# AlibabaResearch/efficientteacher

Measured on AMD Instinct MI355X. Metric: SSOD images/sec (teacher+student step) YOLOv5l 640px, higher is better.
Workload: dtype bf16

## Files before the change

efficientteacher_amd/_lib.py:

```python
import ctypes
import os
from ctypes import c_char_p, c_double, c_float, c_int, c_int64, c_size_t, c_void_p

import torch

_HERE = os.path.dirname(os.path.abspath(__file__))
LIB_PATH = os.environ.get("ET_HIP_LIB") or os.path.join(_HERE, "libet_hip.so")

ET_F32, ET_BF16, ET_F16 = 0, 1, 2

P = c_void_p
SIGNATURES = {
    "et_build_arch": (c_char_p, []),
    "et_abi_version": (c_int, []),
    "et_nms_ssod_workspace_bytes": (c_int, [c_int, c_int, ctypes.POINTER(c_size_t)]),
    "et_nms_workspace_bytes": (c_int, [c_int, c_int, c_int, c_int, c_int, ctypes.POINTER(c_size_t)]),
    "et_nms": (c_int, [P, c_int, c_int, c_int, c_float, c_float, c_int, c_int, ctypes.c_uint64, ctypes.c_uint64, c_int,
                       c_float, c_int, P, P, P, P, P, c_size_t, P]),
    "et_nms_ssod": (c_int, [P, c_int, c_int, c_int, c_float, c_float, c_int, c_int, P, P, P, P, P, c_size_t, P]),
    "et_val_match": (c_int, [P, c_int, P, c_int, c_int, P, c_int, P, c_int, c_int, P, c_int, c_int, c_int, c_int64, c_int64,
                             P, P, P, P, P, P]),
    "et_val_ap_workspace_bytes": (c_int, [c_int, ctypes.POINTER(c_size_t)]),
    "et_val_ap": (c_int, [P, P, P, c_int64, P, c_int, c_int, P, P, P, P, P, c_size_t, P]),
    "et_detect_decode": (c_int, [P, c_int, c_int, c_int, c_int, c_int, c_int, c_int64, c_int64, c_int64, c_int64,
                                 P, c_float, P, c_int64, c_int64, P]),
    "et_ema_update": (c_int, [P, P, c_int64, c_float, c_float, P]),
    "et_adamw": (c_int, [P, P, P, P, P, c_int, c_int64, c_float, c_float, c_float, c_float, c_float, c_int, c_float, P, P]),
    "et_adamw_tick": (c_int, [P, c_float, c_float, P, P]),
    "et_adamw_dev": (c_int, [P, P, P, P, P, c_int, c_int64, c_float, c_float, c_float, c_float, c_float, P, c_float, P, P]),
    "et_sgd_nesterov": (c_int, [P, P, P, P, c_int, c_int64, c_float, c_float, c_float, c_int, c_float, P, P]),
    "et_cast_f32_to_lp": (c_int, [P, P, c_int, c_int64, P]),
    "et_scaler_check": (c_int, [P, c_int64, P, P]),
    "et_scaler_update": (c_int, [P, c_float, c_float, c_int, P]),
    "et_ema_update_dev": (c_int, [P, P, c_int64, P, P]),
    "et_sgd_nesterov_dev": (c_int, [P, P, P, P, c_int, c_int64, P, c_int, P, P]),
    "et_conv2d_stats_rows": (c_int, [c_int, c_int, c_int]),
    "et_conv2d_stats_rows_for": (c_int, [c_int] * 12),
    "et_conv2d_stats_adds_for": (c_int, [c_int] * 12),
    "et_conv2d_fwd": (c_int, [P, P, P, c_int] + [c_int] * 11 + [P, P, c_int, P, c_int, P, c_int, P, P]),
    "et_conv2d_dgrad": (c_int, [P, P, P, c_int] + [c_int] * 11 + [c_int, P, c_int, P, P]),
    "et_conv2d_dgrad_bn": (c_int, [P, P, P, c_int] + [c_int] * 10 + [P, c_int, P, c_int, P, P, c_int, P, c_int, P, P]),
    "et_conv2d_wgrad": (c_int, [P, P, P, c_int] + [c_int] * 11 + [P, P]),
    "et_conv2d_wgrad_grouped": (c_int, [P, c_int, c_int] + [c_int] * 9 + [P, P]),
    "et_weight_transpose_all": (c_int, [P, P, c_int, P, c_int, ctypes.c_longlong, P]),
    "et_weight_transpose": (c_int, [P, P, c_int, c_int, c_int, c_int, P]),
    "et_conv2d_kernel_name": (c_int, [c_int] * 13 + [c_char_p, c_int]),
    "et_env_knobs": (c_int, [c_char_p, c_int]),
    "et_colsum": (c_int, [P, c_int, c_int, c_int, c_int, P, P]),
    "et_bn_reduce_rows": (c_int, [c_int, c_int, c_int]),
    "et_bn_finalize": (c_int, [P, c_int, c_int, c_double, P, P, c_float, c_float, P, P, P, P, P, P, P, P]),
    "et_bn_eval_affine": (c_int, [c_int, P, P, P, P, c_float, P, P, P]),
    "et_bn_act_fwd": (c_int, [P, c_int, P, c_int, P, c_int, c_int, c_int, c_int, P, P, c_int, P]),
    "et_bn_act_fwd_sharded": (c_int, [P, c_int, P, c_int, P, c_int, c_int, c_int, c_int, P, c_int, c_double, P, P, c_float, c_float,
                                      P, P, P, P, P, P, c_int, P]),
    "et_bn_act_bwd_sharded": (c_int, [P, c_int, P, c_int, P, c_int, c_int, c_int, c_int, P, P, P, P, P, c_int, P, P, P, c_int, c_int, P]),
    "et_bn_act_bwd": (c_int, [P, c_int, P, c_int, P, c_int, c_int, c_int, c_int, P, P, P, P, P, c_int, P, P, P, P,
                              c_size_t, P]),
    "et_bn_act_bwd_from_partials": (c_int, [P, c_int, P, c_int, P, c_int, c_int, c_int, c_int, P, P, P, P, P, c_int, P, P, P,
                                            P, c_int, P, P]),
    "et_act_bwd": (c_int, [P, c_int, P, c_int, P, c_int, c_int, c_int, c_int, c_int, P]),
    "et_pack_input": (c_int, [P, P, c_int, c_int, c_int, c_int, c_int, P]),
    "et_pack_input_u8": (c_int, [P, P, c_int, c_int, c_int, c_int, c_int, c_float, P]),
    "et_maxpool5_fwd": (c_int, [P, c_int, P, c_int, P, c_int, c_int, c_int, c_int, c_int, P]),
    "et_maxpool5_bwd": (c_int, [P, c_int, P, P, c_int, P, c_int, c_int, c_int, c_int, c_int, c_int, P]),
    "et_upsample2x_fwd": (c_int, [P, c_int, P, c_int, c_int, c_int, c_int, c_int, c_int, P]),
    "et_upsample2x_bwd": (c_int, [P, c_int, P, c_int, c_int, c_int, c_int, c_int, c_int, c_int, P]),
    "et_strong_view_u8": (c_int, [P, P, c_int, c_int, c_int, P, P, P, P, c_int, P]),
    "et_mosaic4_u8": (c_int, [P, P, c_int, c_int, c_int, P]),
# ... 6 lines not shown
    "et_scale_cast": (c_int, [P, P, c_int, c_int64, c_float, P, P]),
    "et_domain_focal": (c_int, [P, c_int, c_int, c_int64, c_int, c_float, P, c_int, P, P]),
    "et_scale_inplace": (c_int, [P, c_int, c_int64, c_float, P, P]),
    "et_v8_decode": (c_int, [P, c_int, P, c_int, c_int, c_int, c_int, c_int, c_int, c_int, c_float, c_float, P, c_int64, c_int64, P]),
    "et_tal_loss": (c_int, [P, P, P, P, P, P, P, c_int, c_int, c_int, c_int, c_int, c_float, c_float, c_float, P, P, P, P, P]),
    "et_tal_assign_workspace_bytes": (c_int, [c_int, c_int, c_int, ctypes.POINTER(c_size_t)]),
    "et_tal_assign": (c_int, [P, P, P, P, P, P, c_int, c_int, c_int, c_int, c_int, c_float, c_float, c_float, P, P, P, P, P, c_size_t, P]),
    "et_tal_targets_pad": (c_int, [P, c_int, c_int, c_int, c_float, c_float, P, P, P]),
    "et_tal_pseudo_split": (c_int, [P, P, P, P, c_int, c_int, c_int, c_int, c_int, c_int, c_float, c_float, P, P, P, P, P, P, P, P, P]),
    "et_tal_assigned_gt": (c_int, [P, c_int, c_int, c_int, P, P]),
    "et_tal_merge_pseudo": (c_int, [P, P, P, P, P, P, P, P, P, c_int, c_int, c_int, c_int, P, P, P, P]),
}



class WgradItem(ctypes.Structure):
    _fields_ = [("x", ctypes.c_void_p), ("dy", ctypes.c_void_p), ("dw", ctypes.c_void_p), ("ldx", ctypes.c_int),
                ("ldy", ctypes.c_int)]


class LossLevel(ctypes.Structure):
    _fields_ = [("p", P), ("dp", P), ("tobj_ws", P), ("sb", c_int64), ("sa", c_int64), ("sy", c_int64),
                ("sx", c_int64), ("ny", c_int), ("nx", c_int), ("anchors", c_float * 6), ("balance", c_float)]


class LossDesc(ctypes.Structure):
    _fields_ = [("dtype", c_int), ("B", c_int), ("na", c_int), ("nc", c_int), ("NT", c_int), ("nl", c_int),
                ("anchor_t", c_float), ("gr", c_float), ("cp", c_float), ("cn", c_float), ("cls_pw", c_float),
                ("obj_pw", c_float), ("box_w", c_float), ("obj_w", c_float), ("cls_w", c_float),
                ("pass_mask", c_int), ("ignore_obj", c_int), ("targets", P), ("acc_ws", P), ("out", P),
                ("ota_match", P), ("obj_channel", c_int), ("balance_dev", P), ("autobalance_ssi", c_int), ("fl_gamma", c_float), ("level", LossLevel * 4)]


_dll = None
_emulated = False
CALL_TIMER = None
_NO_LAUNCH = frozenset(n for n in (
    "et_build_arch", "et_abi_version", "et_nms_ssod_workspace_bytes", "et_nms_workspace_bytes", "et_conv2d_stats_rows", "et_conv2d_stats_rows_for",
    "et_conv2d_kernel_name", "et_env_knobs", "et_bn_reduce_rows", "et_ota_workspace_bytes", "et_tal_assign_workspace_bytes", "et_val_ap_workspace_bytes"))


class _TimedDll:

    def __init__(self, dll, timer):
        self._dll, self._timer, self._cache = dll, timer, {}

    def __getattr__(self, name):
        fn = self._cache.get(name)
        if fn is None:
            raw = getattr(self._dll, name)
            if name in _NO_LAUNCH or not name.startswith("et_"):
                fn = raw
            else:
                timer = self._timer

                def fn(*a, _raw=raw, _name=name):
                    tok = timer.begin(_name)
                    rc = _raw(*a)
                    timer.end(tok)
                    return rc
            self._cache[name] = fn
        return fn


class EtHipError(RuntimeError):
    pass
# ... 78 lines not shown
```

efficientteacher_amd/csrc/conv.hip:

```cpp
#include "et_device.h"
#include "../../include/et_hip.h"
#include <stdlib.h>
#include <stdio.h>
#include <string.h>
#include <type_traits>

typedef __attribute__((ext_vector_type(16))) float f32x16;
typedef __attribute__((ext_vector_type(8))) __bf16 bf16x8;
typedef __attribute__((ext_vector_type(8))) _Float16 f16x8;
typedef __attribute__((ext_vector_type(4))) unsigned int u32x4;
__device__ __forceinline__ u32x4 mk4(unsigned a, unsigned b, unsigned c, unsigned d) { u32x4 v = {a, b, c, d}; return v; }
__device__ __forceinline__ void et_pin_loaded(u32x4& v) {
#if defined(__HIP_DEVICE_COMPILE__)
    asm volatile("" : "+v"(v));
#endif
}

template <typename T, typename V> __device__ __forceinline__ f32x16 et_mfma32(const V a, const V b, const f32x16 c) {
    static_assert(sizeof(V) == 16, "8 x 16-bit operands");
    if constexpr (std::is_same<T, et_f16>::value)
        return __builtin_amdgcn_mfma_f32_32x32x16_f16(__builtin_bit_cast(f16x8, a), __builtin_bit_cast(f16x8, b), c, 0, 0, 0);
    else
        return __builtin_amdgcn_mfma_f32_32x32x16_bf16(__builtin_bit_cast(bf16x8, a), __builtin_bit_cast(bf16x8, b), c, 0, 0, 0);
}
// ... 3031 lines not shown
extern "C" int et_conv2d_kernel_name(int op, int dtype, int N, int IH, int IW, int Cin, int Cout, int KH, int KW, int stride,
                                     int pad, int have_zero_page, int parity_class, char* buf, int buflen) {
    if (!buf || buflen < 8) return -1;
    if (KH * KW > CONV_MAX_TAPS || stride < 1 || N <= 0) return -2;
    const int eb = dtype == ET_F32 ? 4 : 2, vec = dtype == ET_F32 ? 4 : 8;
    if (op == 2) {
        WgradGeom g;
        wgrad_geom(g, N, IH, IW, Cin, Cin, Cout, KH, KW, stride, pad, Cout);
        wgrad_plan_name(plan_wgrad(g, eb, have_zero_page != 0), dtype, buf, buflen);
        return 0;
    }
    GatherGeom g;
    const bool full = op == 3 || op == 4;
    if (op == 3) op = 1;
    if (op == 4) op = 0;
    if (op == 0) {
        if (!full && try_launch_stem(nullptr, nullptr, nullptr, dtype, N, IH, IW, Cin, Cin, Cout, KH, KW, stride, pad, Cout, nullptr, nullptr, 0,
                                     nullptr, nullptr, 0, have_zero_page ? (const void*)buf : nullptr, nullptr, false)) {
            snprintf(buf, buflen, "conv_stem_kernel");
            return 0;
        }
        if (fwd_geom(g, N, IH, IW, Cin, Cin, Cout, KH, KW, stride, pad, Cout, vec)) return -2;
    } else if (op == 1) {
        if (stride > 2 || Cout % vec) return -2;
        const int py = parity_class / stride, px = parity_class % stride;
        if (py >= stride) return -2;
        if (dgrad_geom(g, py, px, N, IH, IW, Cin, Cin, Cout, KH, KW, stride, pad, Cout, vec)) return -2;
    } else return -2;
    plan_name(plan_gemm(g, eb, have_zero_page != 0, full), dtype, buf, buflen);
    return 0;
}

extern "C" int et_env_knobs(char* buf, int buflen) {
    static const char* names[] = {"ET_CONV_S1_WGS", "ET_CONV_STEM_WGS", "ET_CONV_BUF_DMA", "ET_BN_FIN_SMALL", "ET_STEP_GRAPH", "ET_WGRAD_STREAM",
                                  "ET_ALLREDUCE_CHUNK_MB", "ET_ALLREDUCE_DTYPE", "ET_RCCL_CHANNELS", "ET_DP_SINGLE_RANK", "ET_HIP_LIB"};
    if (!buf || buflen < 1) return -1;
    int off = 0;
    buf[0] = 0;
    for (const char* n : names) {
        const char* v = getenv(n);
        if (!v) continue;
        const int w = snprintf(buf + off, buflen - off, "%s=%s;", n, v);
        if (w < 0 || w >= buflen - off) return -3;
        off += w;
    }
    return 0;
}
```

efficientteacher_amd/csrc/optim.hip:

```cpp
#include "et_device.h"
#include <math.h>
#include "../../include/et_hip.h"

__device__ __forceinline__ uint16_t lp_of(float v, int shadow_dtype) { return shadow_dtype == ET_F16 ? et_f2h(v) : et_f2bf(v); }
#define ET_SCALER_SKIP(scaler) ((scaler) != nullptr && (scaler)[2] != 0.0f)
#define ET_SCALER_INV(scaler) ((scaler) != nullptr ? (scaler)[1] : 1.0f)

__global__ __launch_bounds__(256) void ema_kernel(float* __restrict__ v, const float* __restrict__ m, long long n,
                                                  float d, float omd) {
    const long long i4 = ((long long)blockIdx.x * 256 + threadIdx.x) * 4;
    if (i4 + 3 < n) {
        float4 a = *(float4*)(v + i4);
        const float4 b = *(const float4*)(m + i4);
        a.x = a.x * d; a.x = a.x + omd * b.x;
        a.y = a.y * d; a.y = a.y + omd * b.y;
        a.z = a.z * d; a.z = a.z + omd * b.z;
        a.w = a.w * d; a.w = a.w + omd * b.w;
        *(float4*)(v + i4) = a;
    } else {
        for (long long i = i4; i < n; ++i) { float a = v[i] * d; v[i] = a + omd * m[i]; }
    }
}

extern "C" int et_ema_update(float* ema, const float* model, int64_t n, float d, float one_minus_d,
// ... 65 lines not shown
}

__global__ __launch_bounds__(256) void sgd_kernel(float* __restrict__ p, const float* __restrict__ g,
                                                  float* __restrict__ buf, uint16_t* __restrict__ shadow, int shadow_dtype,
                                                  long long n, float lr, float mu, float wd, int first,
                                                  float inv_scale_host, const float* __restrict__ scaler) {
    if (ET_SCALER_SKIP(scaler)) return;
    const float inv_scale = inv_scale_host * ET_SCALER_INV(scaler);
    const long long i = (long long)blockIdx.x * 256 + threadIdx.x;
    if (i >= n) return;
    float gi = g[i] * inv_scale;
    const float pi = p[i];
    if (wd != 0.0f) gi = gi + wd * pi;
    float b = first ? gi : (buf[i] * mu + gi);
    buf[i] = b;
    gi = gi + mu * b;
    const float o = pi - lr * gi;
    p[i] = o;
    if (shadow) shadow[i] = lp_of(o, shadow_dtype);
}

extern "C" int et_sgd_nesterov(float* p, const float* grad, float* momentum_buf, void* lp_shadow, int shadow_dtype, int64_t n,
                               float lr, float momentum, float weight_decay, int first_step, float inv_scale,
                               const float* scaler, et_stream_t stream) {
    if (!p || !grad || !momentum_buf) return -1;
    if (n < 0 || (lp_shadow && shadow_dtype != ET_BF16 && shadow_dtype != ET_F16)) return -2;
    if (n == 0) return 0;
    hipLaunchKernelGGL(sgd_kernel, dim3(et_cdiv(n, 256)), dim3(256), 0, (hipStream_t)stream, p, grad, momentum_buf,
                       (uint16_t*)lp_shadow, shadow_dtype, (long long)n, lr, momentum, weight_decay, first_step, inv_scale, scaler);
    ET_CHECK_LAUNCH();
    return 0;
}

template <bool DEV>
__global__ __launch_bounds__(256) void adamw_kernel(float* __restrict__ p, const float* __restrict__ g, float* __restrict__ m,
                                                    float* __restrict__ v, uint16_t* __restrict__ shadow, int shadow_dtype, long long n,
                                                    float lr_wd, float b1, float b2, float step_size, float inv_sqrt_bc2, float eps,
                                                    float inv_scale_host, const float* __restrict__ scaler, float lr,
                                                    const double* __restrict__ tick) {
    if (ET_SCALER_SKIP(scaler)) return;
    if constexpr (DEV) {
        step_size = (float)((double)lr / tick[1]);
        inv_sqrt_bc2 = (float)(1.0 / sqrt(tick[2]));
    }
    const float inv_scale = inv_scale_host * ET_SCALER_INV(scaler);
    const long long i = (long long)blockIdx.x * 256 + threadIdx.x;
    if (i >= n) return;
    const float gi = g[i] * inv_scale;
    float pi = p[i];
    pi = pi * (1.0f - lr_wd);
    float mi = m[i];
    mi = mi + (gi - mi) * (1.0f - b1);
    float vi = v[i] * b2;
    vi = vi + (1.0f - b2) * gi * gi;
    const float denom = sqrtf(vi) * inv_sqrt_bc2 + eps;
    pi = pi - step_size * (mi / denom);
    p[i] = pi; m[i] = mi; v[i] = vi;
    if (shadow) shadow[i] = lp_of(pi, shadow_dtype);
}

extern "C" int et_adamw(float* p, const float* grad, float* exp_avg, float* exp_avg_sq, void* lp_shadow, int shadow_dtype, int64_t n,
                        float lr, float beta1, float beta2, float eps, float weight_decay, int step, float inv_scale,
                        const float* scaler, et_stream_t stream) {
    if (!p || !grad || !exp_avg || !exp_avg_sq) return -1;
    if (n < 0 || step < 1 || (lp_shadow && shadow_dtype != ET_BF16 && shadow_dtype != ET_F16)) return -2;
    if (n == 0) return 0;
// ... 109 lines not shown
```

efficientteacher_amd/ops.py:

```python
import torch

from . import _lib
from ._lib import ET_BF16, ET_F16, ET_F32

ACT_NONE, ACT_SILU, ACT_RELU = 0, 1, 2


class KernelTimer:

    def __init__(self):
        self.rows = []
        self.shapes = []

    def span(self, tag, flops, launches=1, nbytes=0, shape=None):
        a, b = torch.cuda.Event(enable_timing=True), torch.cuda.Event(enable_timing=True)
        self.rows.append((tag, flops, launches, nbytes, a, b))
        self.shapes.append(shape)
        return a, b

    def summary(self):
        agg = {}
        for tag, fl, n, nb, a, b in self.rows:
            ms = a.elapsed_time(b)
            t = agg.setdefault(tag, dict(ms=0.0, flops=0.0, launches=0, bytes=0.0))
            t["ms"] += ms; t["flops"] += fl; t["launches"] += n; t["bytes"] += nb
        return agg


TIMER = None
SCOPE = None


class FamilyTimer:

    FAMILY = {
        "et_conv2d_fwd": "gather_gemm", "et_conv2d_dgrad": "gather_gemm", "et_conv2d_dgrad_bn": "gather_gemm",
        "et_conv2d_wgrad": "wgrad", "et_conv2d_wgrad_grouped": "wgrad",
        "et_bn_finalize": "bn", "et_bn_act_fwd": "bn", "et_bn_act_fwd_sharded": "bn", "et_bn_act_bwd_sharded": "bn", "et_bn_act_bwd": "bn", "et_bn_act_bwd_from_partials": "bn", "et_act_bwd": "bn",
        "et_nms": "nms_loss_pl", "et_nms_ssod": "nms_loss_pl", "et_detect_decode": "nms_loss_pl", "et_pseudo_label_transform": "nms_loss_pl",
        "et_select_targets": "nms_loss_pl", "et_yolo_loss": "nms_loss_pl", "et_ota_assign": "nms_loss_pl", "et_score_log_append": "nms_loss_pl",
        "et_scale_cast": "nms_loss_pl", "et_domain_focal": "nms_loss_pl", "et_scale_inplace": "nms_loss_pl", "et_v8_decode": "nms_loss_pl",
        "et_tal_loss": "nms_loss_pl", "et_tal_assign": "nms_loss_pl", "et_colsum": "nms_loss_pl", "et_tal_pseudo_split": "nms_loss_pl", "et_tal_targets_pad": "nms_loss_pl",
        "et_tal_assigned_gt": "nms_loss_pl", "et_tal_merge_pseudo": "nms_loss_pl",
        "et_sgd_nesterov": "optimizer_ema", "et_sgd_nesterov_dev": "optimizer_ema", "et_adamw": "optimizer_ema", "et_ema_update": "optimizer_ema",
        "et_ema_update_dev": "optimizer_ema", "et_cast_f32_to_lp": "optimizer_ema", "et_scaler_check": "optimizer_ema", "et_scaler_update": "optimizer_ema", "et_weight_transpose": "optimizer_ema",
        "et_weight_transpose_all": "optimizer_ema", "et_bn_eval_affine": "optimizer_ema",
    }

    def __init__(self):
        self.rows = []

    def begin(self, name):
        fam = self.FAMILY.get(name, "pool_upsample_pack")
        if fam == "gather_gemm":
            fam = "gather_gemm_teacher" if SCOPE == "teacher" else "gather_gemm_student"
        a, b = torch.cuda.Event(enable_timing=True), torch.cuda.Event(enable_timing=True)
        a.record()
        return (fam, torch.cuda.current_stream().cuda_stream, a, b)

    def end(self, tok):
        tok[3].record()
        self.rows.append(tok)

    def summary(self):
        out = {}
        for fam, sid, a, b in self.rows:
            d = out.setdefault(sid, {})
            d[fam] = d.get(fam, 0.0) + a.elapsed_time(b)
        return out


def kernel_name(op, dtype, N, IH, IW, Cin, Cout, k, stride, pad, parity_class=0, zero_page=True):
    import ctypes
    buf = ctypes.create_string_buffer(256)
    code = {"fwd": 0, "dgrad": 1, "wgrad": 2, "dgrad_full": 3, "fwd_res": 4}[op]
    dt = _ET_OF[dtype]
    _lib.check(_lib.load().et_conv2d_kernel_name(code, dt, N, IH, IW, Cin, Cout, k, k, stride, pad, int(bool(zero_page)),
# ... 728 lines not shown
def _shadow_dt(shadow):
    return et_dtype(shadow) if shadow is not None else ET_BF16


def sgd_nesterov_dev(p, g, buf, shadow, hp, first_step, scaler=None):
    assert hp.dtype == torch.float32 and hp.numel() >= 4
    _lib.check(_lib.load().et_sgd_nesterov_dev(_lib.ptr(p), _lib.ptr(g), _lib.ptr(buf), _lib.ptr(shadow), _shadow_dt(shadow), p.numel(),
                                               _lib.ptr(hp), int(bool(first_step)), _lib.ptr(scaler), _lib.stream(p)), "et_sgd_nesterov_dev")


def adamw(p, g, exp_avg, exp_avg_sq, shadow, lr, beta1, beta2, eps, weight_decay, step, inv_scale=1.0, scaler=None):
    _lib.check(_lib.load().et_adamw(_lib.ptr(p), _lib.ptr(g), _lib.ptr(exp_avg), _lib.ptr(exp_avg_sq), _lib.ptr(shadow), _shadow_dt(shadow),
                                    p.numel(), float(lr), float(beta1), float(beta2), float(eps), float(weight_decay), int(step),
                                    float(inv_scale), _lib.ptr(scaler), _lib.stream(p)), "et_adamw")


def adamw_tick(tick, beta1, beta2, scaler):
    assert tick.dtype == torch.float64 and tick.numel() == 3
    _lib.check(_lib.load().et_adamw_tick(_lib.ptr(tick), float(beta1), float(beta2), _lib.ptr(scaler), _lib.stream(tick)), "et_adamw_tick")


def adamw_dev(p, g, exp_avg, exp_avg_sq, shadow, lr, beta1, beta2, eps, weight_decay, tick, inv_scale=1.0, scaler=None):
    _lib.check(_lib.load().et_adamw_dev(_lib.ptr(p), _lib.ptr(g), _lib.ptr(exp_avg), _lib.ptr(exp_avg_sq), _lib.ptr(shadow), _shadow_dt(shadow),
                                        p.numel(), float(lr), float(beta1), float(beta2), float(eps), float(weight_decay), _lib.ptr(tick),
                                        float(inv_scale), _lib.ptr(scaler), _lib.stream(p)), "et_adamw_dev")


def sgd_nesterov(p, g, buf, shadow, lr, momentum, weight_decay, first_step, inv_scale=1.0, scaler=None):
    _lib.check(_lib.load().et_sgd_nesterov(_lib.ptr(p), _lib.ptr(g), _lib.ptr(buf), _lib.ptr(shadow), _shadow_dt(shadow), p.numel(),
                                           float(lr), float(momentum), float(weight_decay), int(bool(first_step)),
                                           float(inv_scale), _lib.ptr(scaler), _lib.stream(p)), "et_sgd_nesterov")


def detect_decode(raw5, anchor_px, stride, z, a_offset):
    B, na, ny, nx, no = raw5.shape
    assert raw5.stride(4) == 1 and z.is_contiguous() and z.dtype == torch.float32
    _lib.check(_lib.load().et_detect_decode(_lib.ptr(raw5), et_dtype(raw5), B, na, ny, nx, no, raw5.stride(0),
                                            raw5.stride(1), raw5.stride(2), raw5.stride(3), _lib.ptr(anchor_px),
                                            float(stride), _lib.ptr(z), z.shape[1], a_offset, _lib.stream(z)),
               "et_detect_decode")


def domain_focal(feat_nhwc, label, gscale, loss_sum, want_grad=True):
    N, H, W, CP = feat_nhwc.shape
    g = torch.zeros_like(feat_nhwc) if want_grad else None
    _lib.check(_lib.load().et_domain_focal(_lib.ptr(feat_nhwc), _nhwc(feat_nhwc), et_dtype(feat_nhwc), N * H * W, int(label),
                                           float(gscale), _lib.ptr(g), _nhwc(g) if g is not None else 0,
                                           _lib.ptr(loss_sum), _lib.stream(feat_nhwc)), "et_domain_focal")
    return g


def scale_inplace(x, alpha, dev_scale=None):
    assert x.is_contiguous()
    _lib.check(_lib.load().et_scale_inplace(_lib.ptr(x), et_dtype(x), x.numel(), float(alpha), _lib.ptr(dev_scale),
                                            _lib.stream(x)), "et_scale_inplace")
    return x


def v8_decode(reg_nhwc, cls_nhwc, reg_max, nc, stride, cell_offset, out, a_offset):
    B, H, W, _ = reg_nhwc.shape
    assert cls_nhwc.shape[:3] == (B, H, W) and out.is_contiguous() and out.dtype == torch.float32 and reg_nhwc.dtype == cls_nhwc.dtype
    _lib.check(_lib.load().et_v8_decode(_lib.ptr(reg_nhwc), _nhwc(reg_nhwc), _lib.ptr(cls_nhwc), _nhwc(cls_nhwc), et_dtype(reg_nhwc),
                                        B, H, W, int(reg_max), int(nc), float(stride), float(cell_offset), _lib.ptr(out), out.shape[1],
                                        int(a_offset), _lib.stream(out)), "et_v8_decode")


# ... 116 lines not shown
```

efficientteacher_amd/optim.py:

```python
import torch

from . import ops


class DeviceGradScaler:

    def __init__(self, device, enabled=True, init_scale=65536.0, growth_factor=2.0, backoff_factor=0.5, growth_interval=2000):
        self.enabled = bool(enabled)
        self.growth_factor, self.backoff_factor, self.growth_interval = float(growth_factor), float(backoff_factor), int(growth_interval)
        self.state = torch.tensor([init_scale, 1.0 / init_scale, 0.0, 0.0], dtype=torch.float32, device=device) if self.enabled else None

    def scale(self, loss):
        return loss * self.state[0] if self.enabled else loss

    def step(self, optimizer):
        if not self.enabled:
            return optimizer.step()
        ops.WGRAD_QUEUE.join()
        ops.scaler_check(optimizer.flat.grads, self.state)
        return optimizer.step(scaler=self.state)

    def update(self):
        if self.enabled:
            ops.scaler_update(self.state, self.growth_factor, self.backoff_factor, self.growth_interval)

    def get_scale(self):
        return float(self.state[0]) if self.enabled else 1.0

    def state_dict(self):
        return dict(state=self.state.detach().cpu().clone()) if self.enabled else {}

    def load_state_dict(self, sd):
        if self.enabled and "state" in sd:
            self.state.copy_(sd["state"].to(self.state.device))


class FlatSGD(torch.optim.Optimizer):
    def __init__(self, model, lr, momentum=0.937, nesterov=True, weight_decay=0.0):
        if not nesterov:
            raise NotImplementedError("the reference always builds SGD(nesterov=True) (trainer.py:215)")
        self.flat = model.flat_state()
        g_bnw, g_w, g_b = [], [], []
        import torch.nn as nn
        for v in model.modules():
            if hasattr(v, 'bias') and isinstance(v.bias, nn.Parameter):
                g_b.append(v.bias)
            if isinstance(v, nn.BatchNorm2d):
                g_bnw.append(v.weight)
            elif hasattr(v, 'weight') and isinstance(v.weight, nn.Parameter):
                g_w.append(v.weight)
        groups = [dict(params=g_b), dict(params=g_w, weight_decay=weight_decay), dict(params=g_bnw)]
        super().__init__(groups, dict(lr=lr, momentum=momentum, nesterov=True, weight_decay=0.0))
        for g, r in zip(self.param_groups, self.flat.group_ranges()):
            g['range'] = r
            g.setdefault('initial_lr', lr)
        self._model = model
        self.momentum_buf = torch.zeros_like(self.flat.params)
        self.first = True
        self.hp_dev = None
        self.capturing = False

    def state_dict(self):
        sd = super().state_dict()
        sd["flat_momentum"] = self.momentum_buf.detach().cpu().clone()
        sd["flat_first"] = bool(self.first)
        return sd

    def load_state_dict(self, sd):
        sd = dict(sd)
        mom, first = sd.pop("flat_momentum", None), sd.pop("flat_first", None)
        if mom is None:
            raise ValueError("not a FlatSGD state_dict (no flat momentum arena)")
        if mom.numel() != self.momentum_buf.numel():
            raise ValueError("flat momentum arena of another model layout")
        ranges = [g["range"] for g in self.param_groups]
        super().load_state_dict(sd)
        for g, r in zip(self.param_groups, ranges):
            g["range"] = r
        self.momentum_buf.copy_(mom.to(self.momentum_buf.device))
        self.first = bool(first)

    @torch.no_grad()
    def step(self, closure=None, inv_scale=1.0, scaler=None):
        f = self.flat
        if f is not self._model.flat_state():
            raise RuntimeError("the model's arenas were rebuilt (model.to() / set_compute_dtype() / _apply) after this optimizer "
                               "was created: it would update orphaned buffers -- build the optimizer after the last such call")
        assert not ops.WGRAD_QUEUE.pending, "weight gradients still queued: backward() did not finish"
        ops.WGRAD_QUEUE.join()
        for j, g in enumerate(self.param_groups):
            o, n = g['range']
            shadow = f.shadow if (f.shadow is not None and (o, n) == tuple(f.w_range)) else None
            if self.capturing and self.hp_dev is not None:
                ops.sgd_nesterov_dev(f.params[o:o + n], f.grads[o:o + n], self.momentum_buf[o:o + n], shadow, self.hp_dev[j],
                                     self.first, scaler)
            else:
                ops.sgd_nesterov(f.params[o:o + n], f.grads[o:o + n], self.momentum_buf[o:o + n], shadow,
                                 g['lr'], g['momentum'], g['weight_decay'], self.first, inv_scale, scaler)
        self.first = False
        f.w_version += 1

    def hp_values(self, inv_scale=1.0):
        out = []
        for g in self.param_groups:
            out += [float(g['lr']), float(g['momentum']), float(g['weight_decay']), float(inv_scale)]
        return out

    def zero_grad(self, set_to_none=False):
        self.flat.zero_grad()


class FlatAdamW(torch.optim.Optimizer):

    def __init__(self, model, lr, betas=(0.9, 0.999), eps=1e-8, weight_decay=0.0, default_weight_decay=1e-2):
        import torch.nn as nn
        self.flat = model.flat_state()
        g_bnw, g_w, g_b = [], [], []
        for v in model.modules():
            if hasattr(v, 'bias') and isinstance(v.bias, nn.Parameter):
                g_b.append(v.bias)
            if isinstance(v, nn.BatchNorm2d):
                g_bnw.append(v.weight)
# ... 70 lines not shown
```

efficientteacher_amd/trainer/ssod_trainer.py:

```python
from contextlib import nullcontext as _nullcontext

import torch

from ..models.loss import DomainLoss, TargetLoss, build_ssod_loss
from ..parallel import FlatDataParallel
from ..utils.self_supervised_utils import FairPseudoLabel
from ..utils.torch_utils import CosineEMA, SemiSupModelEMA
from .trainer import Trainer


class SSODTrainer(Trainer):
    MODEL_MODULE = "efficientteacher_amd.models.detector.yolo_ssod"

    def __init__(self, cfg, device, callbacks=None, LOCAL_RANK=-1, RANK=-1, WORLD_SIZE=1, nb=1000, target_data_len=None,
                 label_num_per_image=None, cls_ratio_gt=None, amp_dtype=None):
        self.cfg = cfg
        self._amp_dtype_arg = amp_dtype
        self.set_env(cfg, device, LOCAL_RANK, RANK, WORLD_SIZE, callbacks, nb)
        self.build_model(cfg, device)
        self.build_optimizer(cfg)
        if cfg.SSOD.pseudo_label_type == 'FairPseudoLabel':
            self.pseudo_label_creator = FairPseudoLabel(cfg)
        elif cfg.SSOD.pseudo_label_type == 'LabelMatch':
            from ..utils.labelmatch import LabelMatch
            if cls_ratio_gt is None:
                raise ValueError("LabelMatch needs target_data_len, label_num_per_image and cls_ratio_gt (ssod_trainer.py:71)")
            self.pseudo_label_creator = LabelMatch(cfg, int(target_data_len / WORLD_SIZE), label_num_per_image,
                                                   cls_ratio_gt=cls_ratio_gt)
        else:
            raise NotImplementedError(f"SSOD.pseudo_label_type {cfg.SSOD.pseudo_label_type}")
        self.build_ddp_model(cfg, device)

    def after_epoch(self, epoch=None):
        epoch = self.epoch if epoch is None else epoch
        if self.cfg.SSOD.pseudo_label_type == 'LabelMatch' and epoch >= self.cfg.SSOD.dynamic_thres_epoch:
            self.pseudo_label_creator.update_epoch_cls_thr(epoch - self.start_epoch)
            self.compute_un_sup_loss.ignore_thres_high = self.pseudo_label_creator.cls_thr_high
            self.compute_un_sup_loss.ignore_thres_low = self.pseudo_label_creator.cls_thr_low

    def set_env(self, cfg, device, LOCAL_RANK, RANK, WORLD_SIZE, callbacks, nb=1000):
# ... 8 lines not shown
        self.teacher_after = "p3"
        self._side = None
        import os
        self.use_graph = os.environ.get("ET_STEP_GRAPH", "0") == "1"
        self.graph_warmup = 3
        self._eager_steps = 0
        self._capturing = False
        self._graph = None
        self.graph_error = None
        self._strong_view = None

    def _side_stream(self):
        if self._side is None:
            self._side = torch.cuda.Stream(device=self.device)
        return self._side

    def build_model(self, cfg, device):
        super().build_model(cfg, device)
        if cfg.hyp.burn_epochs > 0:
            self.semi_ema = None
        elif self.cosine_ema:
            self.semi_ema = CosineEMA(self.ema.ema, decay_start=cfg.SSOD.ema_rate, total_epoch=self.epochs)
        else:
            self.semi_ema = SemiSupModelEMA(self.ema.ema, cfg.SSOD.ema_rate)

    def build_ddp_model(self, cfg, device):
        super().build_ddp_model(cfg, device)
        self.compute_un_sup_loss = build_ssod_loss(self.model, cfg)
        self.domain_loss = DomainLoss()
        self.target_loss = TargetLoss()

    join_teacher_late = True

    def update_optimizer(self, loss, ni):
        self.scaler.scale(loss).backward()
        if self._capturing:
            if isinstance(self.model, FlatDataParallel):
                self.model.reduce_gradients()
            self.scaler.step(self.optimizer)
            self.scaler.update()
            self.optimizer.zero_grad()
            self.ema.update(self.model)
            if self.semi_ema:
                self.semi_ema.update(self.ema.ema)
            return
        if isinstance(self.model, FlatDataParallel):
            self.model.reduce_gradients()
        self.accumulate = 1 if self.fixed_accumulate else max(round(64 / self.batch_size), 1)
        self._warmup(ni, 1 if self.fixed_accumulate else 64 / self.batch_size)
        if ni - self.last_opt_step >= self.accumulate:
            self.scaler.step(self.optimizer)
            self.scaler.update()
            self.optimizer.zero_grad()
            self.ema.update(self.model)
            if self.semi_ema:
                self.semi_ema.update(self.ema.ema)
            self.last_opt_step = ni

    @staticmethod
    def split_predict_and_feature(total_pred, total_feature, n_img):
        sup_feature = [f[:n_img] for f in total_feature]
        un_sup_feature = [f[n_img:] for f in total_feature]
        if isinstance(total_pred, tuple) and len(total_pred) == 3 and isinstance(total_pred[0], (list, tuple)):
            feats, cls, reg = total_pred
            return (([f[:n_img] for f in feats], cls[:n_img], reg[:n_img]), sup_feature,
                    ([f[n_img:] for f in feats], cls[n_img:], reg[n_img:]), un_sup_feature)
        from ..autograd import split_batch
        halves = [split_batch(p, n_img) for p in total_pred]
        sup_pred = [h[0] for h in halves]
        un_sup_pred = [h[1] for h in halves]
        return sup_pred, sup_feature, un_sup_pred, un_sup_feature

    def train_instance(self, imgs, targets, paths, unlabeled_imgs, unlabeled_imgs_ori, unlabeled_gt, unlabeled_M, ni,
                       pbar=None, callbacks=None):
        if self.use_graph and self._graph_capable() and self._eager_steps >= self.graph_warmup:
            accumulate = 1 if self.fixed_accumulate else max(round(64 / self.batch_size), 1)
            if ni <= self.nw and not self.fixed_accumulate:
                import numpy as np
                accumulate = max(1, np.interp(ni, [0, self.nw], [1, 64 / self.batch_size]).round())
            if self._graph is None:
                from .graph_step import StepGraph
                self._graph = StepGraph(self)
            if accumulate == 1 and self._graph.usable(imgs, targets):
                try:
                    return self._graph.run(imgs, targets, unlabeled_imgs, unlabeled_imgs_ori, unlabeled_M, ni)
                except Exception as e:
                    if self._graph.graph is not None:
                        raise
                    import logging
# ... 124 lines not shown
```

efficientteacher_amd/utils/torch_utils.py:

```python
import math
from copy import deepcopy

import numpy as np
import torch
import torch.nn as nn

from .. import ops


def is_parallel(model):
    from ..parallel import FlatDataParallel
    return type(model) in (nn.parallel.DataParallel, nn.parallel.DistributedDataParallel, FlatDataParallel)


def de_parallel(model):
    return model.module if is_parallel(model) else model


def copy_attr(a, b, include=(), exclude=()):
    wanted = set(include)
    for name, value in vars(b).items():
        if name.startswith('_') or name in exclude or (wanted and name not in wanted):
            continue
        setattr(a, name, value)


def initialize_weights(model):
    for m in model.modules():
        if type(m) is nn.BatchNorm2d:
            m.eps, m.momentum = 1e-3, 0.03


def _flat_ema_update(ema_model, model, d, d_dev=None):
    src = de_parallel(model)
    fe, fm = ema_model.flat_state(), src.flat_state()
    if d_dev is not None:
        ops.ema_update_dev(fe.params, fm.params, d_dev)
        ops.ema_update_dev(fe.buffers, fm.buffers, d_dev)
    else:
        ops.ema_update(fe.params, fm.params, d)
        ops.ema_update(fe.buffers, fm.buffers, d)
    fe.mark_weights_changed()


class _EMABase:
    d_dev = None
    capturing = False

    def _make(self, model):
        self.ema = deepcopy(de_parallel(model)).eval()
        for p in self.ema.parameters():
            p.requires_grad_(False)

    def advance(self):
        raise NotImplementedError

    def update(self, model):
        with torch.no_grad():
            d = None if self.capturing else self.advance()
            _flat_ema_update(self.ema, model, d, self.d_dev if self.capturing else None)

    def update_attr(self, model, include=(), exclude=('process_group', 'reducer')):
        copy_attr(self.ema, model, include, exclude)


class ModelEMA(_EMABase):

    def __init__(self, model, decay=0.9999, updates=0):
        self._make(model)
        self.updates = updates
        self.decay = lambda x: decay * (1 - math.exp(-x / 2000))

    def advance(self):
        self.updates += 1
        return self.decay(self.updates)
# ... 31 lines not shown
```

include/et_hip.h:

```cpp
#ifndef ET_HIP_H
#define ET_HIP_H
#include <stddef.h>
#include <stdint.h>

#ifdef __cplusplus
extern "C" {
#endif

typedef void* et_stream_t;

enum { ET_F32 = 0, ET_BF16 = 1, ET_F16 = 2 };

#define ET_ABI_VERSION 7
const char* et_build_arch(void);
int et_abi_version(void);

int et_nms_ssod_workspace_bytes(int B, int A, size_t* bytes );
int et_nms_ssod(const float* pred, int B, int A, int no, float conf_thres, float iou_thres,
                int agnostic, int max_det, float* dets, int* counts, int64_t* keep,
                int* n_candidates, void* workspace, size_t ws_bytes, et_stream_t stream);

int et_nms_workspace_bytes(int B, int A, int no, int multi_label, int max_nms, size_t* bytes );
int et_nms(const float* pred, int B, int A, int no, float conf_thres, float iou_thres, int agnostic,
           int multi_label, uint64_t class_mask_lo, uint64_t class_mask_hi, int max_nms, float max_wh,
           int max_det, float* dets, int* counts, int64_t* keep, int* n_candidates, void* workspace,
           size_t ws_bytes, et_stream_t stream);

int et_val_match(const float* dets, int det_row_stride, const int* counts, int B, int max_det, const float* targets, int NT,
                 const float* shapes, int net_h, int net_w, const float* iouv, int niou, int single_cls, int nc,
                 int64_t row_offset, int64_t arena_rows, int* correct, float* conf, int* cls, int* valid, int* nt,
                 et_stream_t stream);

int et_val_ap_workspace_bytes(int nc, size_t* bytes );
int et_val_ap(const int* cls, const int* correct, const float* conf, int64_t N, const int* nt, int nc, int niou, double* ap,
              double* p, double* r, double* f1, void* workspace, size_t ws_bytes, et_stream_t stream);

int et_detect_decode(const void* raw, int dtype, int B, int na, int ny, int nx, int no,
                     int64_t sb, int64_t sa, int64_t sy, int64_t sx, const float* anchor_px,
                     float stride, float* z, int64_t A_total, int64_t a_offset, et_stream_t stream);

int et_ema_update(float* ema, const float* model, int64_t n, float d, float one_minus_d, et_stream_t stream);
int et_adamw(float* p, const float* grad, float* exp_avg, float* exp_avg_sq, void* lp_shadow, int shadow_dtype, int64_t n, float lr,
             float beta1, float beta2, float eps, float weight_decay, int step, float inv_scale, const float* scaler,
             et_stream_t stream);
int et_adamw_tick(double* tick, float beta1, float beta2, const float* scaler, et_stream_t stream);
int et_adamw_dev(float* p, const float* grad, float* exp_avg, float* exp_avg_sq, void* lp_shadow, int shadow_dtype, int64_t n, float lr,
                 float beta1, float beta2, float eps, float weight_decay, const double* tick, float inv_scale, const float* scaler,
                 et_stream_t stream);
int et_sgd_nesterov(float* p, const float* grad, float* momentum_buf, void* lp_shadow, int shadow_dtype, int64_t n,
                    float lr, float momentum, float weight_decay, int first_step, float inv_scale, const float* scaler,
                    et_stream_t stream);
int et_cast_f32_to_lp(const float* src, void* dst, int dtype, int64_t n, et_stream_t stream);
int et_scaler_check(const float* grads, int64_t n, float* scaler, et_stream_t stream);
int et_scaler_update(float* scaler, float growth_factor, float backoff_factor, int growth_interval, et_stream_t stream);
int et_ema_update_dev(float* ema, const float* model, int64_t n, const float* d_and_one_minus_d, et_stream_t stream);
int et_sgd_nesterov_dev(float* p, const float* grad, float* momentum_buf, void* lp_shadow, int shadow_dtype, int64_t n,
                        const float* hp, int first_step, const float* scaler, et_stream_t stream);

int et_conv2d_stats_rows(int N, int OH, int OW);
int et_conv2d_stats_rows_for(int op, int dtype, int N, int IH, int IW, int Cin, int Cout, int KH, int KW, int stride, int pad,
                             int have_zero_page);
int et_conv2d_stats_adds_for(int op, int dtype, int N, int IH, int IW, int Cin, int Cout, int KH, int KW, int stride, int pad,
                             int have_zero_page);
#define ET_BN_SHARDS 16
int et_conv2d_fwd(const void* x, const void* w, void* y, int dtype, int N, int IH, int IW, int Cin,
                  int ldx, int Cout, int KH, int KW, int stride, int pad, int ldy, const float* scale,
                  const float* bias, int act, const void* residual, int ldr, float* stats_partial, int stats_ld,
                  const void* zero16, et_stream_t stream);
int et_conv2d_dgrad(const void* dy, const void* wT, void* dx, int dtype, int N, int IH, int IW, int Cin,
                    int ldx, int Cout, int KH, int KW, int stride, int pad, int ldy, int accumulate,
                    const void* residual , int ldr,
                    const void* zero16, et_stream_t stream);
int et_conv2d_dgrad_bn(const void* dy, const void* wT, void* dx, int dtype, int N, int IH, int IW, int Cin, int ldx, int Cout,
                       int KH, int KW, int pad, int ldy, const void* residual, int ldr, const void* bn_y, int ld_bn,
                       const float* bn_scale, const float* bn_shift, int bn_act, float* bn_stats_partial,
                       int bn_stats_ld ,
                       const void* zero16, et_stream_t stream);
int et_conv2d_wgrad(const void* x, const void* dy, float* dw, int dtype, int N, int IH, int IW, int Cin,
                    int ldx, int Cout, int KH, int KW, int stride, int pad, int ldy, const void* zero16,
                    et_stream_t stream);
typedef struct et_wgrad_item { const void* x; const void* dy; float* dw; int ldx, ldy; } et_wgrad_item;
int et_conv2d_wgrad_grouped(const et_wgrad_item* items , int n_items, int dtype, int N, int IH, int IW,
                            int Cin, int Cout, int KH, int KW, int stride, int pad, const void* zero16,
                            et_stream_t stream);
int et_weight_transpose(const void* w, void* wT, int dtype, int Cout, int taps, int Cin, et_stream_t stream);
int et_conv2d_kernel_name(int op, int dtype, int N, int IH, int IW, int Cin, int Cout, int KH, int KW, int stride,
                          int pad, int have_zero_page, int parity_class, char* buf , int buflen);
int et_env_knobs(char* buf , int buflen);
int et_weight_transpose_all(const void* w_arena, void* wT_arena, int dtype, const int* table, int n_layers,
                            long long total_elems, et_stream_t stream);
// ... 117 lines not shown
```

Before: 1325.

## Fuse SGD Nesterov step with teacher and semi EMA updates into one kernel

Adds a single elementwise kernel that applies the per-group SGD Nesterov update, writes the low-precision weight shadow, then updates the teacher EMA and second-level semi EMA (plus its shadow) in the same pass. Buffer EMAs are handled in a second call. This replaces several separate passes over the parameter arenas, cutting repeated reads of the updated params and extra kernel launches. The change adds descriptor plumbing, eligibility checks, and a per-element group lookup, and changes where EMA weights are marked dirty.

After: 1329, median of 6. About the same (+0.3%).

```diff
diff --git a/efficientteacher_amd/_lib.py b/efficientteacher_amd/_lib.py
--- a/efficientteacher_amd/_lib.py
+++ b/efficientteacher_amd/_lib.py
@@ -34,6 +34,7 @@
     "et_scaler_update": (c_int, [P, c_float, c_float, c_int, P]),
     "et_ema_update_dev": (c_int, [P, P, c_int64, P, P]),
     "et_sgd_nesterov_dev": (c_int, [P, P, P, P, c_int, c_int64, P, c_int, P, P]),
+    "et_sgd_ema_tail": (c_int, [P, P]),
     "et_conv2d_stats_rows": (c_int, [c_int, c_int, c_int]),
     "et_conv2d_stats_rows_for": (c_int, [c_int] * 12),
     "et_conv2d_stats_adds_for": (c_int, [c_int] * 12),
@@ -106,6 +107,13 @@
                 ("ota_match", P), ("obj_channel", c_int), ("balance_dev", P), ("autobalance_ssi", c_int), ("fl_gamma", c_float), ("level", LossLevel * 4)]
 
 
+class TailDesc(ctypes.Structure):
+    _fields_ = [("p", P), ("grad", P), ("momentum_buf", P), ("shadow", P), ("ema_shadow", P), ("ema", P), ("semi_ema", P),
+                ("n", c_int64), ("w_off", c_int64), ("w_n", c_int64), ("group_end", c_int64 * 4), ("hp", (c_float * 4) * 4),
+                ("hp_dev", P), ("ema_d", c_float * 2), ("semi_d", c_float * 2), ("ema_d_dev", P), ("semi_d_dev", P),
+                ("scaler", P), ("n_groups", c_int), ("first_step", c_int), ("shadow_dtype", c_int)]
+
+
 _dll = None
 _emulated = False
 CALL_TIMER = None
diff --git a/efficientteacher_amd/csrc/conv.hip b/efficientteacher_amd/csrc/conv.hip
--- a/efficientteacher_amd/csrc/conv.hip
+++ b/efficientteacher_amd/csrc/conv.hip
@@ -3087,7 +3087,7 @@
 }
 
 extern "C" int et_env_knobs(char* buf, int buflen) {
-    static const char* names[] = {"ET_CONV_S1_WGS", "ET_CONV_STEM_WGS", "ET_CONV_BUF_DMA", "ET_BN_FIN_SMALL", "ET_STEP_GRAPH", "ET_WGRAD_STREAM",
+    static const char* names[] = {"ET_CONV_S1_WGS", "ET_CONV_STEM_WGS", "ET_CONV_BUF_DMA", "ET_BN_FIN_SMALL", "ET_STEP_GRAPH", "ET_WGRAD_STREAM", "ET_FUSED_TAIL",
                                   "ET_ALLREDUCE_CHUNK_MB", "ET_ALLREDUCE_DTYPE", "ET_RCCL_CHANNELS", "ET_DP_SINGLE_RANK", "ET_HIP_LIB"};
     if (!buf || buflen < 1) return -1;
     int off = 0;
diff --git a/efficientteacher_amd/csrc/optim.hip b/efficientteacher_amd/csrc/optim.hip
--- a/efficientteacher_amd/csrc/optim.hip
+++ b/efficientteacher_amd/csrc/optim.hip
@@ -121,6 +121,110 @@
     return 0;
 }
 
+struct tail_args {
+    float* p; const float* g; float* buf;
+    uint16_t* shadow; uint16_t* ema_shadow;
+    float* ema; float* semi;
+    long long n, w_off, w_n;
+    long long group_end[ET_TAIL_MAX_GROUPS];
+    float hp[ET_TAIL_MAX_GROUPS][4];
+    const float* hp_dev;
+    float ema_d[2], semi_d[2];
+    const float* ema_d_dev; const float* semi_d_dev;
+    const float* scaler;
+    int n_groups, first, shadow_dtype;
+};
+
+__device__ __forceinline__ void tail_store_lp(uint16_t* dst, const float4 v, int dtype) {
+    *(uint2*)dst = dtype == ET_F16 ? make_uint2(et_pack_h2(v.x, v.y), et_pack_h2(v.z, v.w))
+                                   : make_uint2(et_pack_bf2(v.x, v.y), et_pack_bf2(v.z, v.w));
+}
+__device__ __forceinline__ float tail_sgd1(float pi, float g, float& m, float lr, float mu, float wd, float inv_scale, int first) {
+    float gi = g * inv_scale;
+    if (wd != 0.0f) gi = gi + wd * pi;
+    const float b = first ? gi : (m * mu + gi);
+    m = b;
+    gi = gi + mu * b;
+    return pi - lr * gi;
+}
+__device__ __forceinline__ float tail_ema1(float v, float m, float d, float omd) { const float a = v * d; return a + omd * m; }
+
+__global__ __launch_bounds__(256) void sgd_ema_tail_kernel(const tail_args a) {
+    const long long i = ((long long)blockIdx.x * 256 + threadIdx.x) * 4;
+    if (i >= a.n) return;
+    float4 p = *(const float4*)(a.p + i);
+    const bool in_w = i >= a.w_off && i < a.w_off + a.w_n;
+    if (a.g != nullptr && !ET_SCALER_SKIP(a.scaler)) {
+        float lr = 0.f, mu = 0.f, wd = 0.f, inv_scale = 0.f;
+#pragma unroll
+        for (int j = 0; j < ET_TAIL_MAX_GROUPS; ++j)
+            if (j < a.n_groups && (j == 0 || i >= a.group_end[j > 0 ? j - 1 : 0])) {
+                if (a.hp_dev != nullptr) { lr = a.hp_dev[4 * j]; mu = a.hp_dev[4 * j + 1]; wd = a.hp_dev[4 * j + 2]; inv_scale = a.hp_dev[4 * j + 3]; }
+                else { lr = a.hp[j][0]; mu = a.hp[j][1]; wd = a.hp[j][2]; inv_scale = a.hp[j][3]; }
+            }
+        inv_scale = inv_scale * ET_SCALER_INV(a.scaler);
+        const float4 g = *(const float4*)(a.g + i);
+        float4 m = make_float4(0.f, 0.f, 0.f, 0.f);
+        if (!a.first) m = *(const float4*)(a.buf + i);
+        p.x = tail_sgd1(p.x, g.x, m.x, lr, mu, wd, inv_scale, a.first);
+        p.y = tail_sgd1(p.y, g.y, m.y, lr, mu, wd, inv_scale, a.first);
+        p.z = tail_sgd1(p.z, g.z, m.z, lr, mu, wd, inv_scale, a.first);
+        p.w = tail_sgd1(p.w, g.w, m.w, lr, mu, wd, inv_scale, a.first);
+        *(float4*)(a.buf + i) = m;
+        *(float4*)(a.p + i) = p;
+        if (a.shadow != nullptr && in_w) tail_store_lp(a.shadow + (i - a.w_off), p, a.shadow_dtype);
+    }
+    if (a.ema == nullptr) return;
+    const float d = a.ema_d_dev != nullptr ? a.ema_d_dev[0] : a.ema_d[0], omd = a.ema_d_dev != nullptr ? a.ema_d_dev[1] : a.ema_d[1];
+    float4 e = *(const float4*)(a.ema + i);
+    e.x = tail_ema1(e.x, p.x, d, omd); e.y = tail_ema1(e.y, p.y, d, omd);
+    e.z = tail_ema1(e.z, p.z, d, omd); e.w = tail_ema1(e.w, p.w, d, omd);
+    *(float4*)(a.ema + i) = e;
+    if (a.ema_shadow != nullptr && in_w) tail_store_lp(a.ema_shadow + (i - a.w_off), e, a.shadow_dtype);
+    if (a.semi == nullptr) return;
+    const float d2 = a.semi_d_dev != nullptr ? a.semi_d_dev[0] : a.semi_d[0], omd2 = a.semi_d_dev != nullptr ? a.semi_d_dev[1] : a.semi_d[1];
+    float4 s = *(const float4*)(a.semi + i);
+    s.x = tail_ema1(s.x, e.x, d2, omd2); s.y = tail_ema1(s.y, e.y, d2, omd2);
+    s.z = tail_ema1(s.z, e.z, d2, omd2); s.w = tail_ema1(s.w, e.w, d2, omd2);
+    *(float4*)(a.semi + i) = s;
+}
+
+extern "C" int et_sgd_ema_tail(const et_tail_desc* t, et_stream_t stream) {
+    if (!t || !t->p) return -1;
+    if (t->grad && (!t->momentum_buf || (!t->hp_dev && t->n_groups < 1))) return -1;
+    if (!t->grad && !t->ema) return -1;
+    if (t->semi_ema && !t->ema) return -2;
+    if (t->n < 0 || (t->n & 3) || t->n_groups < 0 || t->n_groups > ET_TAIL_MAX_GROUPS) return -2;
+    const bool lp = t->shadow || t->ema_shadow;
+    if (lp && (t->shadow_dtype != ET_BF16 && t->shadow_dtype != ET_F16)) return -2;
+    if (lp && (t->w_off < 0 || t->w_n < 0 || t->w_off + t->w_n > t->n || (t->w_off & 3) || (t->w_n & 3))) return -2;
+    if (t->shadow && !t->grad) return -2;
+    if (t->ema_shadow && !t->ema) return -2;
+    if ((((uintptr_t)t->p | (uintptr_t)t->grad | (uintptr_t)t->momentum_buf | (uintptr_t)t->ema | (uintptr_t)t->semi_ema) & 15) ||
+        (((uintptr_t)t->shadow | (uintptr_t)t->ema_shadow) & 7)) return -2;
+    tail_args a;
+    a.p = t->p; a.g = t->grad; a.buf = t->momentum_buf; a.shadow = (uint16_t*)t->shadow; a.ema_shadow = (uint16_t*)t->ema_shadow;
+    a.ema = t->ema; a.semi = t->semi_ema;
+    a.n = t->n; a.w_off = lp ? t->w_off : 0; a.w_n = lp ? t->w_n : 0;
+    a.n_groups = t->grad ? t->n_groups : 0;
+    long long prev = 0;
+    for (int j = 0; j < ET_TAIL_MAX_GROUPS; ++j) {
+        const bool used = j < a.n_groups;
+        if (used && (t->group_end[j] < prev || t->group_end[j] > t->n || (t->group_end[j] & 3))) return -2;
+        a.group_end[j] = used ? (prev = t->group_end[j]) : t->n;
+        for (int k = 0; k < 4; ++k) a.hp[j][k] = used ? t->hp[j][k] : 0.0f;
+    }
+    if (a.n_groups > 0 && a.group_end[a.n_groups - 1] != t->n) return -2;
+    a.hp_dev = t->hp_dev;
+    a.ema_d[0] = t->ema_d[0]; a.ema_d[1] = t->ema_d[1]; a.semi_d[0] = t->semi_d[0]; a.semi_d[1] = t->semi_d[1];
+    a.ema_d_dev = t->ema_d_dev; a.semi_d_dev = t->semi_d_dev;
+    a.scaler = t->scaler; a.first = t->first_step != 0; a.shadow_dtype = t->shadow_dtype;
+    if (t->n == 0) return 0;
+    hipLaunchKernelGGL(sgd_ema_tail_kernel, dim3(et_cdiv(t->n, 1024)), dim3(256), 0, (hipStream_t)stream, a);
+    ET_CHECK_LAUNCH();
+    return 0;
+}
+
 template <bool DEV>
 __global__ __launch_bounds__(256) void adamw_kernel(float* __restrict__ p, const float* __restrict__ g, float* __restrict__ m,
                                                     float* __restrict__ v, uint16_t* __restrict__ shadow, int shadow_dtype, long long n,
diff --git a/efficientteacher_amd/ops.py b/efficientteacher_amd/ops.py
--- a/efficientteacher_amd/ops.py
+++ b/efficientteacher_amd/ops.py
@@ -42,7 +42,7 @@
         "et_scale_cast": "nms_loss_pl", "et_domain_focal": "nms_loss_pl", "et_scale_inplace": "nms_loss_pl", "et_v8_decode": "nms_loss_pl",
         "et_tal_loss": "nms_loss_pl", "et_tal_assign": "nms_loss_pl", "et_colsum": "nms_loss_pl", "et_tal_pseudo_split": "nms_loss_pl", "et_tal_targets_pad": "nms_loss_pl",
         "et_tal_assigned_gt": "nms_loss_pl", "et_tal_merge_pseudo": "nms_loss_pl",
-        "et_sgd_nesterov": "optimizer_ema", "et_sgd_nesterov_dev": "optimizer_ema", "et_adamw": "optimizer_ema", "et_ema_update": "optimizer_ema",
+        "et_sgd_nesterov": "optimizer_ema", "et_sgd_nesterov_dev": "optimizer_ema", "et_sgd_ema_tail": "optimizer_ema", "et_adamw": "optimizer_ema", "et_ema_update": "optimizer_ema",
         "et_ema_update_dev": "optimizer_ema", "et_cast_f32_to_lp": "optimizer_ema", "et_scaler_check": "optimizer_ema", "et_scaler_update": "optimizer_ema", "et_weight_transpose": "optimizer_ema",
         "et_weight_transpose_all": "optimizer_ema", "et_bn_eval_affine": "optimizer_ema",
     }
@@ -837,6 +837,34 @@
                                            float(inv_scale), _lib.ptr(scaler), _lib.stream(p)), "et_sgd_nesterov")
 
 
+def sgd_ema_tail(p, g, buf, shadow, groups, first_step, scaler, emas, w_range, hp_dev=None):
+    import ctypes
+    assert p.dtype == torch.float32 and 1 <= len(emas) + (g is not None) and len(emas) <= 2 and len(groups) <= 4
+    t = _lib.TailDesc()
+    t.p, t.grad, t.momentum_buf, t.shadow = _lib.ptr(p), _lib.ptr(g), _lib.ptr(buf), _lib.ptr(shadow)
+    t.n, t.w_off, t.w_n = p.numel(), int(w_range[0]), int(w_range[1])
+    lp = shadow
+    for k, (arena, d, d_dev, e_shadow) in enumerate(emas):
+        assert arena.dtype == torch.float32 and arena.numel() == p.numel() and (k == 0 or e_shadow is None)
+        pair = (0.0, 0.0) if d is None else (float(d), float(1. - d))
+        assert d is not None or d_dev is not None
+        if k == 0:
+            t.ema, t.ema_d[0], t.ema_d[1], t.ema_d_dev, t.ema_shadow = _lib.ptr(arena), pair[0], pair[1], _lib.ptr(d_dev), _lib.ptr(e_shadow)
+            lp = e_shadow if e_shadow is not None else lp
+        else:
+            t.semi_ema, t.semi_d[0], t.semi_d[1], t.semi_d_dev = _lib.ptr(arena), pair[0], pair[1], _lib.ptr(d_dev)
+    if shadow is not None and emas and emas[0][3] is not None:
+        assert shadow.dtype == emas[0][3].dtype
+    assert lp is None or lp.numel() == t.w_n
+    t.shadow_dtype = _shadow_dt(lp)
+    t.n_groups, t.first_step, t.hp_dev, t.scaler = len(groups), int(bool(first_step)), _lib.ptr(hp_dev), _lib.ptr(scaler)
+    for j, (end, *hp) in enumerate(groups):
+        t.group_end[j] = int(end)
+        for k in range(4):
+            t.hp[j][k] = float(hp[k])
+    _lib.check(_lib.load().et_sgd_ema_tail(ctypes.byref(t), _lib.stream(p)), "et_sgd_ema_tail")
+
+
 def detect_decode(raw5, anchor_px, stride, z, a_offset):
     B, na, ny, nx, no = raw5.shape
     assert raw5.stride(4) == 1 and z.is_contiguous() and z.dtype == torch.float32
diff --git a/efficientteacher_amd/optim.py b/efficientteacher_amd/optim.py
--- a/efficientteacher_amd/optim.py
+++ b/efficientteacher_amd/optim.py
@@ -1,6 +1,10 @@
+import os
+
 import torch
 
 from . import ops
+
+FUSED_TAIL = os.environ.get("ET_FUSED_TAIL", "1") != "0"
 
 
 class DeviceGradScaler:
@@ -13,12 +17,12 @@
     def scale(self, loss):
         return loss * self.state[0] if self.enabled else loss
 
-    def step(self, optimizer):
+    def step(self, optimizer, **kw):
         if not self.enabled:
-            return optimizer.step()
+            return optimizer.step(**kw)
         ops.WGRAD_QUEUE.join()
         ops.scaler_check(optimizer.flat.grads, self.state)
-        return optimizer.step(scaler=self.state)
+        return optimizer.step(scaler=self.state, **kw)
 
     def update(self):
         if self.enabled:
@@ -80,14 +84,31 @@
         self.momentum_buf.copy_(mom.to(self.momentum_buf.device))
         self.first = bool(first)
 
+    def groups_tile_arena(self):
+        end = 0
+        for g in self.param_groups:
+            o, n = g['range']
+            if o != end or n % 4:
+                return False
+            end = o + n
+        return end == self.flat.params.numel() and len(self.param_groups) <= 4
+
     @torch.no_grad()
-    def step(self, closure=None, inv_scale=1.0, scaler=None):
+    def step(self, closure=None, inv_scale=1.0, scaler=None, emas=None):
         f = self.flat
         if f is not self._model.flat_state():
             raise RuntimeError("the model's arenas were rebuilt (model.to() / set_compute_dtype() / _apply) after this optimizer "
                                "was created: it would update orphaned buffers -- build the optimizer after the last such call")
         assert not ops.WGRAD_QUEUE.pending, "weight gradients still queued: backward() did not finish"
         ops.WGRAD_QUEUE.join()
+        if emas:
+            dev = self.capturing and self.hp_dev is not None
+            groups = [(g['range'][0] + g['range'][1], g['lr'], g['momentum'], g['weight_decay'], inv_scale) for g in self.param_groups]
+            ops.sgd_ema_tail(f.params, f.grads, self.momentum_buf, f.shadow, groups, self.first, scaler, emas, f.w_range,
+                             hp_dev=self.hp_dev if dev else None)
+            self.first = False
+            f.w_version += 1
+            return
         for j, g in enumerate(self.param_groups):
             o, n = g['range']
             shadow = f.shadow if (f.shadow is not None and (o, n) == tuple(f.w_range)) else None
diff --git a/efficientteacher_amd/trainer/ssod_trainer.py b/efficientteacher_amd/trainer/ssod_trainer.py
--- a/efficientteacher_amd/trainer/ssod_trainer.py
+++ b/efficientteacher_amd/trainer/ssod_trainer.py
@@ -5,7 +5,7 @@
 from ..models.loss import DomainLoss, TargetLoss, build_ssod_loss
 from ..parallel import FlatDataParallel
 from ..utils.self_supervised_utils import FairPseudoLabel
-from ..utils.torch_utils import CosineEMA, SemiSupModelEMA
+from ..utils.torch_utils import CosineEMA, SemiSupModelEMA, fused_tail
 from .trainer import Trainer
 
 
@@ -80,29 +80,34 @@
 
     join_teacher_late = True
 
+    def _step_and_emas(self):
+        tail = fused_tail(self.model, self.optimizer, [self.ema, self.semi_ema]) if self.ema else None
+        if tail is not None:
+            self.scaler.step(self.optimizer, emas=tail.begin())
+            self.scaler.update()
+            self.optimizer.zero_grad()
+            tail.finish()
+            return
+        self.scaler.step(self.optimizer)
+        self.scaler.update()
+        self.optimizer.zero_grad()
+        self.ema.update(self.model)
+        if self.semi_ema:
+            self.semi_ema.update(self.ema.ema)
+
     def update_optimizer(self, loss, ni):
         self.scaler.scale(loss).backward()
         if self._capturing:
             if isinstance(self.model, FlatDataParallel):
                 self.model.reduce_gradients()
-            self.scaler.step(self.optimizer)
-            self.scaler.update()
-            self.optimizer.zero_grad()
-            self.ema.update(self.model)
-            if self.semi_ema:
-                self.semi_ema.update(self.ema.ema)
+            self._step_and_emas()
             return
         if isinstance(self.model, FlatDataParallel):
             self.model.reduce_gradients()
         self.accumulate = 1 if self.fixed_accumulate else max(round(64 / self.batch_size), 1)
         self._warmup(ni, 1 if self.fixed_accumulate else 64 / self.batch_size)
         if ni - self.last_opt_step >= self.accumulate:
-            self.scaler.step(self.optimizer)
-            self.scaler.update()
-            self.optimizer.zero_grad()
-            self.ema.update(self.model)
-            if self.semi_ema:
-                self.semi_ema.update(self.ema.ema)
+            self._step_and_emas()
             self.last_opt_step = ni
 
     @staticmethod
diff --git a/efficientteacher_amd/utils/torch_utils.py b/efficientteacher_amd/utils/torch_utils.py
--- a/efficientteacher_amd/utils/torch_utils.py
+++ b/efficientteacher_amd/utils/torch_utils.py
@@ -41,6 +41,45 @@
         ops.ema_update(fe.params, fm.params, d)
         ops.ema_update(fe.buffers, fm.buffers, d)
     fe.mark_weights_changed()
+
+
+class FusedTail:
+
+    def __init__(self, fm, emas):
+        self.fm, self.emas = fm, emas
+        self.flats = [e.ema.flat_state() for e in emas]
+        self.d = None
+
+    def begin(self):
+        self.d = [(None, e.d_dev) if e.capturing else (e.advance(), None) for e in self.emas]
+        return [(f.params, d, d_dev, f.shadow if k == 0 else None) for k, (f, (d, d_dev)) in enumerate(zip(self.flats, self.d))]
+
+    def finish(self):
+        with torch.no_grad():
+            ops.sgd_ema_tail(self.fm.buffers, None, None, None, [], False, None,
+                             [(f.buffers, d, d_dev, None) for f, (d, d_dev) in zip(self.flats, self.d)], (0, 0))
+        teacher = self.flats[0]
+        teacher.w_version += 1
+        teacher.weights_dirty = False
+        for f in self.flats[1:]:
+            f.mark_weights_changed()
+        self.d = None
+
+
+def fused_tail(model, optimizer, emas):
+    from .. import optim
+    emas = [e for e in emas if e is not None]
+    if not optim.FUSED_TAIL or not isinstance(optimizer, optim.FlatSGD) or not 1 <= len(emas) <= 2:
+        return None
+    fm = de_parallel(model).flat_state()
+    if optimizer.flat is not fm or not optimizer.groups_tile_arena() or fm.buffers.numel() % 4:
+        return None
+    for e in emas:
+        f = e.ema.flat_state()
+        if (f.segments != fm.segments or f.n_params != fm.n_params or f.buffers.numel() != fm.buffers.numel()
+                or f.compute_dtype != fm.compute_dtype or f.params.device != fm.params.device):
+            return None
+    return FusedTail(fm, emas)
 
 
 class _EMABase:
diff --git a/include/et_hip.h b/include/et_hip.h
--- a/include/et_hip.h
+++ b/include/et_hip.h
@@ -11,7 +11,7 @@
 
 enum { ET_F32 = 0, ET_BF16 = 1, ET_F16 = 2 };
 
-#define ET_ABI_VERSION 7
+#define ET_ABI_VERSION 8
 const char* et_build_arch(void);
 int et_abi_version(void);
 
@@ -56,6 +56,21 @@
 int et_ema_update_dev(float* ema, const float* model, int64_t n, const float* d_and_one_minus_d, et_stream_t stream);
 int et_sgd_nesterov_dev(float* p, const float* grad, float* momentum_buf, void* lp_shadow, int shadow_dtype, int64_t n,
                         const float* hp, int first_step, const float* scaler, et_stream_t stream);
+#define ET_TAIL_MAX_GROUPS 4
+typedef struct {
+    float* p; const float* grad; float* momentum_buf;
+    void* shadow; void* ema_shadow;
+    float* ema; float* semi_ema;
+    int64_t n, w_off, w_n;
+    int64_t group_end[ET_TAIL_MAX_GROUPS];
+    float hp[ET_TAIL_MAX_GROUPS][4];
+    const float* hp_dev;
+    float ema_d[2], semi_d[2];
+    const float* ema_d_dev; const float* semi_d_dev;
+    const float* scaler;
+    int n_groups, first_step, shadow_dtype;
+} et_tail_desc;
+int et_sgd_ema_tail(const et_tail_desc* desc , et_stream_t stream);
 
 int et_conv2d_stats_rows(int N, int OH, int OW);
 int et_conv2d_stats_rows_for(int op, int dtype, int N, int IH, int IW, int Cin, int Cout, int KH, int KW, int stride, int pad,
```
